# microsoft/GenerativeImage2Text

Hardware: AMD Instinct MI355X
Metric: captions/sec whole-node (GIT_BASE 224px bs=64/GPU greedy len=20) (higher is better)
Workload: dtype f16; 1 GPU; GIT_BASE 224px bs=64/GPU greedy max_len=20 frames=1; global_batch=64, parallelism=dp1, decode_steps_per_caption=19, seq_len_returned=20, hip_graph=True, contexts_in_flight=4, layernorm_folded=True, library=libgitmi_f16.so, encoder_chains=2, schedule=mixed

## Files before the change

### generativeimage2text_amd/csrc/kernels_attn_decode.hip

```cpp
#include "gitmi_common.h"
#include "launchers.h"
#include "dgemm_shared.h"
#include <algorithm>
#include <type_traits>

#pragma clang fp contract(off)

namespace gitmi {

static constexpr int HD = 64;

__global__ __launch_bounds__(256) void kv_repack_frag_kernel(const bf16_t* __restrict__ qkv, bf16_t* __restrict__ kf,
                                                             bf16_t* __restrict__ vt, int N, int Np, int H, int d) {
    __shared__ bf16_t vs[32][HD + 8];
    const int s = blockIdx.x, h = blockIdx.y, b = blockIdx.z, tid = threadIdx.x;
    const int nsteps = Np >> 5;
    bf16_t* kdst = kf + ((size_t)b * H + h) * Np * HD;
    bf16_t* vdst = vt + ((size_t)b * H + h) * Np * HD;
    const int key = tid >> 3, ch = tid & 7;
    const int n = s * 32 + key;
    u32x4_t kv = {0u, 0u, 0u, 0u}, vv = kv;
    if (n < N) {
        const bf16_t* src = qkv + ((size_t)b * N + n) * 3 * d + d + h * HD + ch * 8;
        kv = *reinterpret_cast<const u32x4_t*>(src);
        vv = *reinterpret_cast<const u32x4_t*>(src + d);
    }
    *reinterpret_cast<u32x4_t*>(kdst + frag_tile(n >> 4, ch >> 2, 2, (ch & 3) * 16 + (n & 15))) = kv;
    *reinterpret_cast<u32x4_t*>(&vs[key][ch * 8]) = vv;
    __syncthreads();
    const int dt = tid >> 6, lane = tid & 63, lg = lane >> 4, dim = dt * 16 + (lane & 15);
    bf16_t o[8];
#pragma unroll
    for (int e = 0; e < 8; ++e) o[e] = vs[(e >> 2) * 16 + lg * 4 + (e & 3)][dim];
    u32x4_t ov;
#pragma unroll
    for (int e = 0; e < 4; ++e) ov[e] = (uint32_t)o[2 * e] | ((uint32_t)o[2 * e + 1] << 16);
    *reinterpret_cast<u32x4_t*>(vdst + (((size_t)s * 4 + dt) * 64 + lane) * 8) = ov;
}

__device__ __forceinline__ void unpack8(const u32x4_t& r, float (&v)[8]) {
#pragma unroll
    for (int i = 0; i < 4; ++i) {
        unpack2op(r[i], v[2 * i], v[2 * i + 1]);
    }
}
__device__ __forceinline__ void ld8bf(const bf16_t* p, float (&v)[8]) { unpack8(*reinterpret_cast<const u32x4_t*>(p), v); }

constexpr int ACS = 4;

struct Pair {
    int h, row0;
    bool on;
};

struct QkvSrc {
    const bf16_t* q0;
    int row_stride, part;
    __device__ __forceinline__ const bf16_t* q(int j) const { return q0 + (size_t)j * row_stride; }
    __device__ __forceinline__ const bf16_t* k(int j) const { return q(j) + part; }
    __device__ __forceinline__ const bf16_t* v(int j) const { return q(j) + 2 * part; }
};
__device__ __forceinline__ QkvSrc qkv_rows(const AttnDecodeArgs& a, const Pair& p) {
    return QkvSrc{reinterpret_cast<const bf16_t*>(a.qkv) + (size_t)p.row0 * (3 * a.d) + p.h * HD, 3 * a.d, a.d};
}

template <int KB>
__device__ __forceinline__ void load_text_kv(const AttnDecodeArgs& a, const Pair& p, const QkvSrc& qs, int j, int s, int sub, u32x4_t& kr, u32x4_t& vr) {
    if (s == a.pos) {
        kr = *reinterpret_cast<const u32x4_t*>(qs.k(j) + sub * 8);
        vr = *reinterpret_cast<const u32x4_t*>(qs.v(j) + sub * 8);
    } else {
        const int srow = KB == 1 ? p.row0 : a.kv_src[(size_t)(p.row0 + j) * a.ld_src + s];
        const size_t off = ((size_t)srow * a.T_max + s) * a.d + p.h * HD + sub * 8;
        kr = *reinterpret_cast<const u32x4_t*>(reinterpret_cast<const bf16_t*>(a.txt_k) + off);
        vr = *reinterpret_cast<const u32x4_t*>(reinterpret_cast<const bf16_t*>(a.txt_v) + off);
    }
}

template <int KB, int TI>
struct TextItems {
    int j[TI];
    u32x4_t kr[TI], vr[TI];
    __device__ __forceinline__ void load(const AttnDecodeArgs& a, const Pair& p, const QkvSrc& qs, int grp, int ngrp, int sub) {
        const int nt = a.pos + 1;
#pragma unroll
        for (int u = 0; u < TI; ++u) {
            const int it = grp + ngrp * u;
            j[u] = (p.on && it < a.beams * nt) ? it / nt : -1;
            const int s = it < a.beams * nt ? it % nt : 0;
            kr[u] = u32x4_t{0u, 0u, 0u, 0u};
            vr[u] = kr[u];
            if (j[u] >= 0) load_text_kv<KB>(a, p, qs, j[u], s, sub, kr[u], vr[u]);
        }
    }
};

__device__ __forceinline__ void append_text_cache(const AttnDecodeArgs& a, const Pair& p, const QkvSrc& qs, int t, int sub) {
    if (p.on && t < a.beams * 8) {
        const int j = t >> 3;
        const size_t dst = ((size_t)(p.row0 + j) * a.T_max + a.pos) * a.d + p.h * HD + sub * 8;
        *reinterpret_cast<u32x4_t*>(reinterpret_cast<bf16_t*>(a.txt_k) + dst) = *reinterpret_cast<const u32x4_t*>(qs.k(j) + sub * 8);
        *reinterpret_cast<u32x4_t*>(reinterpret_cast<bf16_t*>(a.txt_v) + dst) = *reinterpret_cast<const u32x4_t*>(qs.v(j) + sub * 8);
    }
}

__device__ __forceinline__ void load_q_frag(const AttnDecodeArgs& a, const Pair& p, const QkvSrc& qs, int l15, int lg, bf16x8_t (&qf)[2]) {
#pragma unroll
    for (int ds = 0; ds < 2; ++ds) {
        float qv[8] = {0.f, 0.f, 0.f, 0.f, 0.f, 0.f, 0.f, 0.f};
        if (p.on && l15 < a.beams)
            ld8bf(qs.q(l15) + ds * 32 + lg * 8, qv);
        u32x4_t t;
#pragma unroll
        for (int e = 0; e < 4; ++e) t[e] = pack2bf(qv[2 * e] * a.scale, qv[2 * e + 1] * a.scale);
        qf[ds] = __builtin_bit_cast(bf16x8_t, t);
    }
}

struct ImagePartial {
    float m, l;
    f32x4_t o[4];
    __device__ __forceinline__ void init() {
        m = -INFINITY;
        l = 0.f;
#pragma unroll
        for (int dt = 0; dt < 4; ++dt) o[dt] = f32x4_t{0.f, 0.f, 0.f, 0.f};
    }
    __device__ __forceinline__ static void mask_max(f32x4_t (&sc)[2], int s, int nimg_steps, int n_img, int lg, float& cm) {
#pragma unroll
        for (int t = 0; t < 2; ++t)
#pragma unroll
            for (int r = 0; r < 4; ++r) {
                if (s * 32 + t * 16 + lg * 4 + r >= n_img || s >= nimg_steps) sc[t][r] = -INFINITY;
                cm = fmaxf(cm, sc[t][r]);
            }
    }
    __device__ __forceinline__ float new_max(float cm, bool rescale) {
        cm = fmaxf(cm, __shfl_xor(cm, 16, 64));
        cm = fmaxf(cm, __shfl_xor(cm, 32, 64));
        const float mn = fmaxf(m, cm);
        if (rescale) {
            const float al = fast_exp(m - mn);
            l *= al;
#pragma unroll
            for (int dt = 0; dt < 4; ++dt) { o[dt][0] *= al; o[dt][1] *= al; o[dt][2] *= al; o[dt][3] *= al; }
        }
        m = mn;
        return mn;
    }
    __device__ __forceinline__ bf16x8_t p_frag(const f32x4_t (&sc)[2], float mn) {
        float p[8];
#pragma unroll
        for (int t = 0; t < 2; ++t)
#pragma unroll
            for (int r = 0; r < 4; ++r) {
                p[t * 4 + r] = fast_exp(sc[t][r] - mn);
                l += p[t * 4 + r];
            }
        u32x4_t pp;
#pragma unroll
        for (int e = 0; e < 4; ++e) pp[e] = pack2bf(p[2 * e], p[2 * e + 1]);
        return __builtin_bit_cast(bf16x8_t, pp);
    }
    __device__ __forceinline__ void finish() {
        l += __shfl_xor(l, 16, 64);
        l += __shfl_xor(l, 32, 64);
    }
    template <int KB>
    __device__ __forceinline__ void publish(float (&slot)[KB][HD + 2], int k, int l15, int lg) const {
        if (l15 < k) {
#pragma unroll
            for (int dt = 0; dt < 4; ++dt)
#pragma unroll
                for (int r = 0; r < 4; ++r) slot[l15][dt * 16 + lg * 4 + r] = o[dt][r];
            if (lg == 0) { slot[l15][HD] = m; slot[l15][HD + 1] = l; }
        }
    }
};

template <int KB>
struct TextPartial {
    float q[KB][8], m[KB], l[KB], o[KB][8];
    __device__ __forceinline__ void init(const AttnDecodeArgs& a, const Pair& p, const QkvSrc& qs, int sub) {
#pragma unroll
        for (int j = 0; j < KB; ++j) {
            m[j] = -INFINITY;
            l[j] = 0.f;
#pragma unroll
            for (int e = 0; e < 8; ++e) { q[j][e] = 0.f; o[j][e] = 0.f; }
            if (p.on && j < a.beams) {
                ld8bf(qs.q(j) + sub * 8, q[j]);
#pragma unroll
                for (int e = 0; e < 8; ++e) q[j][e] *= a.scale;
            }
        }
    }
    __device__ __forceinline__ void item(int jj, const u32x4_t& kr, const u32x4_t& vr) {
        float kv[8], vv[8];
        unpack8(kr, kv);
        unpack8(vr, vv);
#pragma unroll
        for (int j = 0; j < KB; ++j) {
            if (j == jj) {
                float sv = 0.f;
#pragma unroll
                for (int e = 0; e < 8; ++e) sv = fmaf(q[j][e], kv[e], sv);
                sv += __shfl_xor(sv, 1, 64);
                sv += __shfl_xor(sv, 2, 64);
                sv += __shfl_xor(sv, 4, 64);
                const float mn = fmaxf(m[j], sv);
                const float al = fast_exp(m[j] - mn);
                const float pe = fast_exp(sv - mn);
                l[j] = fmaf(l[j], al, pe);
#pragma unroll
                for (int e = 0; e < 8; ++e) o[j][e] = fmaf(o[j][e], al, pe * vv[e]);
                m[j] = mn;
            }
        }
    }
    template <int TI>
    __device__ __forceinline__ void items(const TextItems<KB, TI>& ti, bool enabled) {
#pragma unroll
        for (int u = 0; u < TI; ++u) {
            if (ti.j[u] >= 0 && enabled) item(ti.j[u], ti.kr[u], ti.vr[u]);
        }
    }
    template <int TI>
    __device__ __forceinline__ void tail(const AttnDecodeArgs& a, const Pair& p, const QkvSrc& qs, int grp, int ngrp, int sub) {
        if (!p.on) return;
        const int nt = a.pos + 1;
        for (int it = grp + ngrp * TI; it < a.beams * nt; it += ngrp) {
            u32x4_t kr, vr;
            load_text_kv<KB>(a, p, qs, it / nt, it % nt, sub, kr, vr);
            item(it / nt, kr, vr);
        }
    }
    __device__ __forceinline__ void merge_groups() {
#pragma unroll
        for (int j = 0; j < KB; ++j) {
#pragma unroll
            for (int off = 8; off < 64; off <<= 1) {
                const float m2 = __shfl_xor(m[j], off, 64);
                const float l2 = __shfl_xor(l[j], off, 64);
                const float mn = fmaxf(m[j], m2);
                const float a1 = m[j] == -INFINITY ? 0.f : fast_exp(m[j] - mn);
                const float a2 = m2 == -INFINITY ? 0.f : fast_exp(m2 - mn);
                l[j] = fmaf(l[j], a1, l2 * a2);
#pragma unroll
                for (int e = 0; e < 8; ++e) {
                    const float o2 = __shfl_xor(o[j][e], off, 64);
                    o[j][e] = fmaf(o[j][e], a1, o2 * a2);
                }
                m[j] = mn;
            }
        }
    }
    __device__ __forceinline__ void fold_into(float (&slot)[KB][HD + 2], int k, int lane, int sub) const {
#pragma unroll
        for (int j = 0; j < KB; ++j) {
            if (lane < 8 && j < k) {
                const float mi = slot[j][HD], li = slot[j][HD + 1];
                const float mn = fmaxf(mi, m[j]);
                const float a1 = mi == -INFINITY ? 0.f : fast_exp(mi - mn);
                const float a2 = m[j] == -INFINITY ? 0.f : fast_exp(m[j] - mn);
#pragma unroll
                for (int e = 0; e < 8; ++e) slot[j][sub * 8 + e] = fmaf(slot[j][sub * 8 + e], a1, o[j][e] * a2);
                if (sub == 0) { slot[j][HD] = mn; slot[j][HD + 1] = fmaf(li, a1, l[j] * a2); }
            }
        }
    }
};

__device__ __forceinline__ void store_out(const AttnDecodeArgs& a, int row, int col, float r) {
    bf16_t* O = reinterpret_cast<bf16_t*>(a.out);
    if (a.out_frag) O[frag_offset(row, col, a.d >> 5)] = f2bf(r);
    else O[(size_t)row * a.d + col] = f2bf(r);
}
template <int KB>
__device__ __forceinline__ void write_rows(const AttnDecodeArgs& a, const Pair& p, const float (&s0)[KB][HD + 2], int t, int nthr) {
    if (!p.on) return;
    for (int i = t; i < a.beams * HD; i += nthr) {
        const int j = i / HD, dd = i % HD;
        const float r1 = s0[j][dd] / s0[j][HD + 1];
        store_out(a, p.row0 + j, p.h * HD + dd, r1);
    }
}
template <int KB>
__device__ __forceinline__ void write_rows(const AttnDecodeArgs& a, const Pair& p, const float (&s0)[KB][HD + 2],
                                           const float (&s1)[KB][HD + 2], int t, int nthr) {
    if (!p.on) return;
    for (int i = t; i < a.beams * HD; i += nthr) {
        const int j = i / HD, dd = i % HD;
        const float m0 = s0[j][HD], m1 = s1[j][HD];
        const float mm = fmaxf(m0, m1);
        const float a0 = m0 == -INFINITY ? 0.f : fast_exp(m0 - mm);
        const float a1 = m1 == -INFINITY ? 0.f : fast_exp(m1 - mm);
        const float num = fmaf(a0, s0[j][dd], a1 * s1[j][dd]);
        const float den = fmaf(a0, s0[j][HD + 1], a1 * s1[j][HD + 1]);
        const float r = num / den;
        store_out(a, p.row0 + j, p.h * HD + dd, r);
    }
}

template <int KB, int TI = 3, int PW = 1, int NH = 2, bool RAGGED = false>
__global__ __launch_bounds__(64 * NH * PW) void attn_decode_mfma_kernel(AttnDecodeArgs a) {
    __shared__ float part[PW][NH][KB][HD + 2];
    constexpr int PT = 64 * NH;

    const int tid = threadIdx.x, lane = tid & 63, wave = tid >> 6;
    const int l15 = lane & 15, lg = lane >> 4;
    const int hp = wave / NH, half = wave % NH;
    const int H = a.d / HD;
    const int k = a.beams;
    const int Np = a.N_pad, nsteps = Np >> 5;
    const int pair = NH == 2 ? (int)(blockIdx.y * H + blockIdx.x) : (int)blockIdx.x * PW + hp;
    Pair p;
    p.on = PW == 1 || pair < a.n_pairs;
    p.h = p.on ? pair % H : 0;
    const int b = p.on ? pair / H : 0;
    p.row0 = b * k;
    const int bi = a.img_of ? a.img_of[b] : b;
    const bf16_t* Kf = reinterpret_cast<const bf16_t*>(a.img_k) + ((size_t)bi * H + p.h) * Np * HD;
    const bf16_t* Vt = reinterpret_cast<const bf16_t*>(a.img_v) + ((size_t)bi * H + p.h) * Np * HD;
    const int n_img = RAGGED ? a.ntok[bi] : a.N_img;
    const int nimg_steps = (!p.on || (a.dbg & 1)) ? 0 : RAGGED ? (n_img + 31) >> 5 : nsteps;

    bf16x8_t kq[ACS][2][2], vq[ACS][4];
    auto load_chunk = [&](int s0) {
#pragma unroll
        for (int c = 0; c < ACS; ++c) {
            const int s = s0 + NH * c;
            const bool on = s < nimg_steps && !(a.dbg & 8);
            const bf16_t* kp = Kf + frag_tile(2 * s, 0, 2, lane);
            const bf16_t* vp = Vt + ((size_t)s * 4 * 64 + lane) * 8;
#pragma unroll
            for (int t = 0; t < 2; ++t)
#pragma unroll
                for (int ds = 0; ds < 2; ++ds) {
                    const bf16x8_t* q = reinterpret_cast<const bf16x8_t*>(kp + (t * 2 + ds) * 512);
                    kq[c][t][ds] = !on ? bf16x8_t{0, 0, 0, 0, 0, 0, 0, 0} : (a.dbg & 16) ? *q : __builtin_nontemporal_load(q);
                }
#pragma unroll
            for (int dt = 0; dt < 4; ++dt) {
                const bf16x8_t* q = reinterpret_cast<const bf16x8_t*>(vp + dt * 512);
                vq[c][dt] = !on ? bf16x8_t{0, 0, 0, 0, 0, 0, 0, 0} : (a.dbg & 16) ? *q : __builtin_nontemporal_load(q);
            }
        }
    };
    load_chunk(half);

    const int t = tid % PT, grp = t >> 3, sub = tid & 7;
    const QkvSrc qs = qkv_rows(a, p);
    TextItems<KB, TI> ti;
    ti.load(a, p, qs, grp, 8 * NH, sub);
    append_text_cache(a, p, qs, t, sub);
    bf16x8_t qf[2];
    load_q_frag(a, p, qs, l15, lg, qf);

    ImagePartial ip;
    ip.init();
    for (int s0 = half; s0 < nimg_steps; s0 += NH * ACS) {
        if (s0 != half) load_chunk(s0);
        f32x4_t sc[ACS][2];
        float cm = -INFINITY;
#pragma unroll
        for (int c = 0; c < ACS; ++c) {
#pragma unroll
            for (int u = 0; u < 2; ++u) {
                sc[c][u] = mfma16(kq[c][u][0], qf[0], f32x4_t{0.f, 0.f, 0.f, 0.f});
                sc[c][u] = mfma16(kq[c][u][1], qf[1], sc[c][u]);
            }
            ip.mask_max(sc[c], s0 + NH * c, nimg_steps, RAGGED ? n_img : a.N_img, lg, cm);
        }
        const float mn = ip.new_max(cm, s0 != half);
#pragma unroll
        for (int c = 0; c < ACS; ++c) {
            const bf16x8_t pf = ip.p_frag(sc[c], mn);
            if (a.dbg & 4) {
#pragma unroll
                for (int dt = 0; dt < 4; ++dt) asm volatile("" ::"v"(vq[c][dt]));
                asm volatile("" ::"v"(pf));
                continue;
            }
#pragma unroll
            for (int dt = 0; dt < 4; ++dt) ip.o[dt] = mfma16(vq[c][dt], pf, ip.o[dt]);
        }
    }
    ip.finish();
    TextPartial<KB> tp;
    tp.init(a, p, qs, sub);
    tp.items(ti, !(a.dbg & 2));
    tp.template tail<TI>(a, p, qs, grp, 8 * NH, sub);
    tp.merge_groups();
    ip.publish(part[hp][half], k, l15, lg);
    if constexpr (NH > 1) __syncthreads(); else __builtin_amdgcn_wave_barrier();
    tp.fold_into(part[hp][half], k, lane, sub);
    if constexpr (NH > 1) __syncthreads(); else __builtin_amdgcn_wave_barrier();
    if constexpr (NH == 1) write_rows(a, p, part[hp][0], t, PT);
    else write_rows(a, p, part[hp][0], part[hp][NH - 1], t, PT);
}

constexpr int AQ_PW = 8;
constexpr int AQ_STRIPS = 3 * HD / 16;

__device__ __forceinline__ void attn_lds_barrier() {
    asm volatile("s_waitcnt lgkmcnt(0)" ::: "memory");
    __builtin_amdgcn_s_barrier();
    asm volatile("" ::: "memory");
}

template <int TI>
__global__ __launch_bounds__(64 * AQ_PW) void attn_decode_qkv_kernel(AttnDecodeArgs a) {
    constexpr int KB = 1;
    __shared__ __attribute__((aligned(16))) f32x4_t red[AQ_STRIPS][4][1][64];
    __shared__ __attribute__((aligned(16))) bf16_t rows[AQ_PW][3 * HD];
    __shared__ float part[AQ_PW][KB][HD + 2];

    const int tid = threadIdx.x, lane = tid & 63;
    const int wave = __builtin_amdgcn_readfirstlane(tid >> 6);
    const int l15 = lane & 15, lg = lane >> 4;
    const int H = a.d / HD, B = a.n_pairs / H;
    const int Np = a.N_pad, nsteps = Np >> 5;
    const int nsb = (B + AQ_PW - 1) / AQ_PW, total = H * nsb, per = (total + 7) >> 3;
    const int blk = (int)(blockIdx.x & 7) * per + (int)(blockIdx.x >> 3);
    if (blk >= total) return;
    const int b0 = (blk % nsb) * AQ_PW;
    Pair p;
    p.h = blk / nsb;
    p.on = b0 + wave < B;
    const int b = p.on ? b0 + wave : 0;
    p.row0 = b;
    const int bi = a.img_of ? a.img_of[b] : b;
    const bf16_t* Kf = reinterpret_cast<const bf16_t*>(a.img_k) + ((size_t)bi * H + p.h) * Np * HD;
    const bf16_t* Vt = reinterpret_cast<const bf16_t*>(a.img_v) + ((size_t)bi * H + p.h) * Np * HD;
    const int nimg_steps = p.on ? nsteps : 0;

    bf16x8_t kq[ACS][2][2], vq[ACS][4];
    auto load_k = [&](int s0) {
#pragma unroll
        for (int c = 0; c < ACS; ++c) {
            const bool on = s0 + c < nimg_steps;
            const bf16_t* kp = Kf + frag_tile(2 * (s0 + c), 0, 2, lane);
#pragma unroll
            for (int t = 0; t < 2; ++t)
#pragma unroll
                for (int ds = 0; ds < 2; ++ds)
                    kq[c][t][ds] = !on ? bf16x8_t{0, 0, 0, 0, 0, 0, 0, 0}
                                       : __builtin_nontemporal_load(reinterpret_cast<const bf16x8_t*>(kp + (t * 2 + ds) * 512));
        }
    };
    auto load_v = [&](int s0) {
#pragma unroll
        for (int c = 0; c < ACS; ++c) {
            const bool on = s0 + c < nimg_steps;
            const bf16_t* vp = Vt + ((size_t)(s0 + c) * 4 * 64 + lane) * 8;
#pragma unroll
            for (int dt = 0; dt < 4; ++dt)
                vq[c][dt] = !on ? bf16x8_t{0, 0, 0, 0, 0, 0, 0, 0}
                                : __builtin_nontemporal_load(reinterpret_cast<const bf16x8_t*>(vp + dt * 512));
        }
    };
    load_k(0);

    const int ksteps = a.d >> 5, N = 3 * a.d;
    const int slice = wave & 3;
    const KSlice ks = k_slice(ksteps, 4, slice);
    const int rt = b0 >> 4;
    auto strip_of = [&](int ls) { return (ls >> 2) * (a.d >> 4) + p.h * 4 + (ls & 3); };
    bf16x8_t xf[DW_KS][1];
    load_x_slice(xf, reinterpret_cast<const bf16_t*>(a.x), rt, ks, ksteps, lane);
#pragma unroll 2
    for (int u = 0; u < AQ_STRIPS / 2; ++u) {
        const int ls = (wave >> 2) * (AQ_STRIPS / 2) + u;
        const WSlice wf = load_w_slice<false>(reinterpret_cast<const bf16_t*>(a.w), strip_of(ls), ks, ksteps, lane);
        f32x4_t acc[1] = {f32x4_t{0.f, 0.f, 0.f, 0.f}};
        mfma_slice(acc, wf, xf, ks);
        red[ls][slice][0][lane] = acc[0];
    }
    load_v(0);
    const int fm_raw = rt * 16 + l15;
    const int fm = fm_raw < a.M ? fm_raw : a.M - 1;
    const bool second = wave + AQ_PW < AQ_STRIPS;
    const int fn0 = strip_of(wave) * 16 + lg * 4, fn1 = strip_of(second ? wave + AQ_PW : wave) * 16 + lg * 4;
    RowStatLoads sl;
    if (a.stats_in) stats_issue(sl, a.stats_in, a.strips_in, a.M, fm, lg);
    const float4 bias4[2] = {load_cols4(a.bias, fn0, N), load_cols4(a.bias, fn1, N)};
    float4 cs4[2] = {float4{0.f, 0.f, 0.f, 0.f}, float4{0.f, 0.f, 0.f, 0.f}};
    if (a.stats_in) { cs4[0] = load_cols4(a.colsum, fn0, N); cs4[1] = load_cols4(a.colsum, fn1, N); }
    attn_lds_barrier();
    {
#pragma clang fp contract(fast)
        float mean = 0.f, rstd = 1.f;
        if (a.stats_in) stats_finish(sl, a.inv_d, a.eps_in, mean, rstd);
        const int i = l15 - (b0 & 15);
#pragma unroll
        for (int t = 0; t < 2; ++t) {
            if (t == 1 && !second) break;
            const int ls = wave + t * AQ_PW;
            const f32x4_t tot = sum_waves<4>(red[ls], 0, lane);
            DGEMM_CONSUMER_FINISH(v, tot, bias4[t], cs4[t], a.stats_in, mean, rstd, GITMI_ACT_NONE);
            if (i >= 0 && i < AQ_PW) {
                uint2 o;
                o.x = pack2bf(v[0], v[1]);
                o.y = pack2bf(v[2], v[3]);
                *reinterpret_cast<uint2*>(&rows[i][ls * 16 + lg * 4]) = o;
            }
        }
    }
    attn_lds_barrier();
    const QkvSrc qs{rows[wave], 0, HD};

    const int grp = lane >> 3, sub = lane & 7;
    TextItems<KB, TI> ti;
    ti.load(a, p, qs, grp, 8, sub);
    append_text_cache(a, p, qs, lane, sub);
    bf16x8_t qf[2];
    load_q_frag(a, p, qs, l15, lg, qf);

    ImagePartial ip;
    ip.init();
    for (int s0 = 0; s0 < nimg_steps; s0 += ACS) {
        if (s0 != 0) { load_k(s0); load_v(s0); }
        f32x4_t sc[ACS][2];
        float cm = -INFINITY;
#pragma unroll
        for (int c = 0; c < ACS; ++c) {
#pragma unroll
            for (int u = 0; u < 2; ++u) {
                sc[c][u] = mfma16(kq[c][u][0], qf[0], f32x4_t{0.f, 0.f, 0.f, 0.f});
                sc[c][u] = mfma16(kq[c][u][1], qf[1], sc[c][u]);
            }
            ip.mask_max(sc[c], s0 + c, nimg_steps, a.N_img, lg, cm);
        }
        const float mn = ip.new_max(cm, s0 != 0);
#pragma unroll
        for (int c = 0; c < ACS; ++c) {
            const bf16x8_t pf = ip.p_frag(sc[c], mn);
#pragma unroll
            for (int dt = 0; dt < 4; ++dt) ip.o[dt] = mfma16(vq[c][dt], pf, ip.o[dt]);
        }
    }
    ip.finish();
    TextPartial<KB> tp;
    tp.init(a, p, qs, sub);
    tp.items(ti, true);
    tp.template tail<TI>(a, p, qs, grp, 8, sub);
    tp.merge_groups();
    ip.publish(part[wave], a.beams, l15, lg);
    __builtin_amdgcn_wave_barrier();
    tp.fold_into(part[wave], a.beams, lane, sub);
    __builtin_amdgcn_wave_barrier();
    write_rows(a, p, part[wave], lane, 64);
}

typedef __attribute__((address_space(3))) void attn_lds_void_t;

template <int N> __device__ __forceinline__ void attn_wait_vm() { asm volatile("s_waitcnt vmcnt(%0)" ::"n"(N) : "memory"); }
__device__ __forceinline__ void attn_wait_slots_ahead(int ahead) {
    switch (ahead) {
        case 0: attn_wait_vm<0>(); break;
        case 1: attn_wait_vm<4>(); break;
        case 2: attn_wait_vm<8>(); break;
        case 3: attn_wait_vm<12>(); break;
        case 4: attn_wait_vm<16>(); break;
        case 5: attn_wait_vm<20>(); break;
        case 6: attn_wait_vm<24>(); break;
        case 7: attn_wait_vm<28>(); break;
        case 8: attn_wait_vm<32>(); break;
        case 9: attn_wait_vm<36>(); break;
        case 10: attn_wait_vm<40>(); break;
        default: attn_wait_vm<44>(); break;
    }
}

constexpr int AS_WAVES = 4;
constexpr int AS_SLOT = 4096;

template <int KB, int TI, int RING>
__global__ __launch_bounds__(64 * AS_WAVES) void attn_decode_stream_kernel(AttnDecodeArgs a) {
    static_assert(RING >= 2 && RING <= 12, "ring depth");
    __shared__ __attribute__((aligned(16))) unsigned char ring_mem[AS_WAVES][RING * AS_SLOT];
    __shared__ float part[AS_WAVES][KB][HD + 2];

    const int tid = threadIdx.x, lane = tid & 63;
    const int wave = __builtin_amdgcn_readfirstlane(tid >> 6);
    const int l15 = lane & 15, lg = lane >> 4;
    const int H = a.d / HD;
    const int k = a.beams;
    const int Np = a.N_pad, nsteps = Np >> 5;
    unsigned char* ring = ring_mem[wave];

    const int W = (int)gridDim.x * AS_WAVES, w0 = (int)blockIdx.x * AS_WAVES + wave;
    const int npw = w0 < a.n_pairs ? (a.n_pairs - 1 - w0) / W + 1 : 0;
    const int slots_per_pair = 2 * nsteps;
    const int total_slots = npw * slots_per_pair;

    int issued = 0;
    int p_ord = 0, p_s0 = 0, p_v = 0, p_c = 0;
    const bf16_t* p_K = nullptr; const bf16_t* p_V = nullptr;
    auto producer_pair = [&]() {
        const int pair = w0 + p_ord * W;
        const int h = pair % H, b = pair / H;
        const int bi = a.img_of ? a.img_of[b] : b;
        p_K = reinterpret_cast<const bf16_t*>(a.img_k) + ((size_t)bi * H + h) * Np * HD;
        p_V = reinterpret_cast<const bf16_t*>(a.img_v) + ((size_t)bi * H + h) * Np * HD;
    };
    if (npw > 0) producer_pair();
    auto issue_slot = [&]() {
        if (issued >= total_slots) return;
        const bf16_t* src = (p_v ? p_V : p_K) + (size_t)(p_s0 + p_c) * (AS_SLOT / 2) + lane * 8;
        unsigned char* dst = ring + (issued % RING) * AS_SLOT;
#pragma unroll
        for (int f = 0; f < 4; ++f)
            __builtin_amdgcn_global_load_lds((const void*)(src + f * 512), (attn_lds_void_t*)(dst + f * 1024), 16, 0, 2);
        ++issued;
        const int nsc = min(ACS, nsteps - p_s0);
        if (++p_c == nsc) {
            p_c = 0;
            if (p_v == 0) p_v = 1;
            else {
                p_v = 0; p_s0 += ACS;
                if (p_s0 >= nsteps) { p_s0 = 0; ++p_ord; if (p_ord < npw) producer_pair(); }
            }
        }
    };
    for (int i = 0; i < RING; ++i) issue_slot();

    int consumed = 0;
    auto slot_ready = [&]() -> const unsigned char* {
        const int ahead = issued - consumed - 1;
        if (ahead == RING - 1) attn_wait_vm<4 * (RING - 1)>();
        else attn_wait_slots_ahead(ahead);
        return ring + (consumed % RING) * AS_SLOT;
    };
    auto slot_done = [&]() {
        asm volatile("s_waitcnt lgkmcnt(0)" ::: "memory");
        ++consumed;
        issue_slot();
    };


    for (int ord = 0; ord < npw; ++ord) {
        const int pair = w0 + ord * W;
        const Pair p{pair % H, (pair / H) * k, true};

        const int grp = lane >> 3, sub = lane & 7;
        const QkvSrc qs = qkv_rows(a, p);
        TextItems<KB, TI> ti;
        ti.load(a, p, qs, grp, 8, sub);
        append_text_cache(a, p, qs, lane, sub);
        bf16x8_t qf[2];
        load_q_frag(a, p, qs, l15, lg, qf);

        ImagePartial ip;
        ip.init();
        for (int s0 = 0; s0 < nsteps; s0 += ACS) {
            f32x4_t sc[ACS][2];
            float cm = -INFINITY;
#pragma unroll
            for (int c = 0; c < ACS; ++c) {
                if (s0 + c < nsteps) {
                    const unsigned char* sl = slot_ready();
                    bf16x8_t kq[2][2];
#pragma unroll
                    for (int t = 0; t < 2; ++t)
#pragma unroll
                        for (int ds = 0; ds < 2; ++ds)
                            kq[t][ds] = *reinterpret_cast<const bf16x8_t*>(sl + (t * 2 + ds) * 1024 + lane * 16);
                    __builtin_amdgcn_sched_barrier(0);
#pragma unroll
                    for (int t = 0; t < 2; ++t) {
                        sc[c][t] = mfma16(kq[t][0], qf[0], f32x4_t{0.f, 0.f, 0.f, 0.f});
                        sc[c][t] = mfma16(kq[t][1], qf[1], sc[c][t]);
                    }
                    slot_done();
                } else {
                    sc[c][0] = f32x4_t{0.f, 0.f, 0.f, 0.f};
                    sc[c][1] = sc[c][0];
                }
                ip.mask_max(sc[c], s0 + c, nsteps, a.N_img, lg, cm);
            }
            const float mn = ip.new_max(cm, s0 != 0);
#pragma unroll
            for (int c = 0; c < ACS; ++c) {
                const bf16x8_t pf = ip.p_frag(sc[c], mn);
                if (s0 + c < nsteps) {
                    const unsigned char* sl = slot_ready();
                    bf16x8_t vq[4];
#pragma unroll
                    for (int dt = 0; dt < 4; ++dt) vq[dt] = *reinterpret_cast<const bf16x8_t*>(sl + dt * 1024 + lane * 16);
                    __builtin_amdgcn_sched_barrier(0);
#pragma unroll
                    for (int dt = 0; dt < 4; ++dt) ip.o[dt] = mfma16(vq[dt], pf, ip.o[dt]);
                    slot_done();
                } else {
#pragma unroll
                    for (int dt = 0; dt < 4; ++dt) ip.o[dt] = mfma16(bf16x8_t{0, 0, 0, 0, 0, 0, 0, 0}, pf, ip.o[dt]);
                }
            }
        }
        ip.finish();
        TextPartial<KB> tp;
        tp.init(a, p, qs, sub);
        tp.items(ti, true);
        tp.template tail<TI>(a, p, qs, grp, 8, sub);
        tp.merge_groups();
        ip.publish(part[wave], k, l15, lg);
        __builtin_amdgcn_wave_barrier();
        tp.fold_into(part[wave], k, lane, sub);
        __builtin_amdgcn_wave_barrier();
        write_rows(a, p, part[wave], lane, 64);
        __builtin_amdgcn_wave_barrier();
    }
}

hipError_t launch_kv_repack_frag(const void* qkv, void* kf, void* vt, int B, int N, int N_pad, int H, int d, hipStream_t s) {
    if (B <= 0 || N <= 0) return hipSuccess;
    if (N_pad % 32 || N_pad < N) return hipErrorInvalidValue;
    hipLaunchKernelGGL(kv_repack_frag_kernel, dim3(N_pad / 32, H, B), dim3(256), 0, s, (const bf16_t*)qkv, (bf16_t*)kf,
                       (bf16_t*)vt, N, N_pad, H, d);
    return hipGetLastError();
}

template <typename F>
static void with_beam_rows(int beams, F&& f) {
    if (beams <= 1) f(std::integral_constant<int, 1>{});
    else if (beams <= 2) f(std::integral_constant<int, 2>{});
    else if (beams <= 4) f(std::integral_constant<int, 4>{});
    else f(std::integral_constant<int, 8>{});
}

int attn_decode_pairs_per_wg(const AttnDecodeArgs& a, int B, int H) {
    int pw = a.pairs_per_wg >= 8 ? 8 : a.pairs_per_wg >= 4 || a.pairs_per_wg <= 0 ? 4 : a.pairs_per_wg >= 2 ? 2 : 1;
    while (pw > 1 && B * H / pw < 96) pw >>= 1;
    if (a.beams > 4 && pw == 8) pw = 4;
    return pw;
}

bool attn_decode_qkv_form(const AttnDecodeArgs& a, int B, int H) {
    if (B <= 0 || a.beams != 1 || a.waves_per_pair == 2 || a.ntok || a.stream_wgs != 0 || a.dbg) return false;
    if (a.N_img < 1 || a.N_pad % 32 || a.N_pad < a.N_img || a.N_pad > 8 * 32) return false;
    if (a.d != H * HD || a.d > 4 * DW_KS * 32 || a.M < B) return false;
    if (!a.x || !a.w || !a.bias) return false;
    return !a.stats_in || (a.colsum && a.strips_in >= 1 && a.strips_in <= 4 * STRIP_SLOTS);
}

hipError_t launch_attn_decode_qkv(const AttnDecodeArgs& a, int B, int H, hipStream_t s) {
    if (!attn_decode_qkv_form(a, B, H)) return hipErrorInvalidValue;
    AttnDecodeArgs p = a;
    p.n_pairs = B * H;
    const int total = H * ((B + AQ_PW - 1) / AQ_PW);
    hipLaunchKernelGGL((attn_decode_qkv_kernel<3>), dim3(8 * ((total + 7) / 8)), dim3(64 * AQ_PW), 0, s, p);
    return hipGetLastError();
}

hipError_t launch_attn_decode_mfma(const AttnDecodeArgs& a, int B, int H, hipStream_t s) {
    if (B <= 0) return hipSuccess;
    if (a.beams > 8 || a.N_pad % 32 || a.N_pad < a.N_img || a.N_img < 1) return hipErrorInvalidValue;
    if (a.ntok && a.stream_wgs > 0) return hipErrorInvalidValue;
    AttnDecodeArgs p = a;
    p.n_pairs = B * H;
    if (a.stream_wgs > 0) {
        const int nwg = std::max(1, std::min(a.stream_wgs, (p.n_pairs + AS_WAVES - 1) / AS_WAVES));
        with_beam_rows(a.beams, [&](auto kb) {
            constexpr int KB = decltype(kb)::value;
            hipLaunchKernelGGL((attn_decode_stream_kernel<KB, 3, KB == 8 ? 8 : 9>), dim3(nwg), dim3(64 * AS_WAVES), 0, s, p);
        });
        return hipGetLastError();
    }
    const bool one_wave = a.waves_per_pair == 1 || (a.waves_per_pair != 2 && a.N_pad <= 8 * 32);
    if (a.ntok || !one_wave) {
        with_beam_rows(a.beams, [&](auto kb) {
            constexpr int KB = decltype(kb)::value;
            if (a.ntok) hipLaunchKernelGGL((attn_decode_mfma_kernel<KB, 3, 1, 2, true>), dim3(H, B), dim3(128), 0, s, p);
            else hipLaunchKernelGGL((attn_decode_mfma_kernel<KB>), dim3(H, B), dim3(128), 0, s, p);
        });
        return hipGetLastError();
    }
    const int pw = attn_decode_pairs_per_wg(a, B, H);
    with_beam_rows(a.beams, [&](auto kb) {
        constexpr int KB = decltype(kb)::value;
        auto packed = [&](auto pwc) {
            constexpr int PW = decltype(pwc)::value;
            hipLaunchKernelGGL((attn_decode_mfma_kernel<KB, 3, PW, 1>), dim3((p.n_pairs + PW - 1) / PW), dim3(64 * PW), 0, s, p);
        };
        if (pw == 8) { if constexpr (KB < 8) packed(std::integral_constant<int, 8>{}); }
        else if (pw == 4) packed(std::integral_constant<int, 4>{});
        else if (pw == 2) packed(std::integral_constant<int, 2>{});
        else packed(std::integral_constant<int, 1>{});
    });
    return hipGetLastError();
}

}
```

Measured before the change: 11700 captions/s.

## Overlap first K/V chunk loads with fused QKV projection via LDS DMA

In the fused QKV-projection plus decode-attention kernel, the first image K chunk is now prefetched. Part of it is DMA'd straight into per-wave LDS slots through global_load_lds, and the rest is loaded into registers, all issued before the projection MFMAs. The W slices and epilogue constants are also hoisted ahead of those MFMAs. Loads for out-of-range steps are always issued against a dummy address, so fixed vmcnt waits can be used, and the results are masked to zero at use. The aim is to hide global latency of K/V behind the GEMM, at the cost of extra LDS (8 waves × 3 × 4KB), more live registers and more complex wait accounting.

```diff
diff --git a/generativeimage2text_amd/csrc/kernels_attn_decode.hip b/generativeimage2text_amd/csrc/kernels_attn_decode.hip
--- a/generativeimage2text_amd/csrc/kernels_attn_decode.hip
+++ b/generativeimage2text_amd/csrc/kernels_attn_decode.hip
@@ -402,6 +402,19 @@
 
 constexpr int AQ_PW = 8;
 constexpr int AQ_STRIPS = 3 * HD / 16;
+constexpr int AQ_LDS_STEPS = 3;
+constexpr int AS_SLOT = 4096;
+typedef __attribute__((address_space(3))) void attn_lds_void_t;
+
+template <int N>
+__device__ __forceinline__ void attn_wait_vm_only() {
+    static_assert(N >= 0 && N < 64, "vmcnt is a 6-bit counter");
+    __builtin_amdgcn_sched_barrier(0);
+    asm volatile("" ::: "memory");
+    __builtin_amdgcn_s_waitcnt((N & 15) | ((N >> 4) << 14) | (7 << 4) | (15 << 8));
+    asm volatile("" ::: "memory");
+    __builtin_amdgcn_sched_barrier(0);
+}
 
 __device__ __forceinline__ void attn_lds_barrier() {
     asm volatile("s_waitcnt lgkmcnt(0)" ::: "memory");
@@ -409,12 +422,14 @@
     asm volatile("" ::: "memory");
 }
 
-template <int TI>
+template <int TI, bool OVL = true>
 __global__ __launch_bounds__(64 * AQ_PW) void attn_decode_qkv_kernel(AttnDecodeArgs a) {
     constexpr int KB = 1;
+    static_assert(AQ_LDS_STEPS < ACS, "the chunk's last step stays in registers");
     __shared__ __attribute__((aligned(16))) f32x4_t red[AQ_STRIPS][4][1][64];
     __shared__ __attribute__((aligned(16))) bf16_t rows[AQ_PW][3 * HD];
     __shared__ float part[AQ_PW][KB][HD + 2];
+    __shared__ __attribute__((aligned(16))) unsigned char kslot[OVL ? AQ_PW : 1][OVL ? AQ_LDS_STEPS * AS_SLOT : 16];
 
     const int tid = threadIdx.x, lane = tid & 63;
     const int wave = __builtin_amdgcn_readfirstlane(tid >> 6);
@@ -436,57 +451,109 @@
     const int nimg_steps = p.on ? nsteps : 0;
 
     bf16x8_t kq[ACS][2][2], vq[ACS][4];
-    auto load_k = [&](int s0) {
-#pragma unroll
-        for (int c = 0; c < ACS; ++c) {
+    const bf16x8_t zero8 = {0, 0, 0, 0, 0, 0, 0, 0};
+    auto load_frag = [&](const bf16_t* q, bool on, auto always_issue) -> bf16x8_t {
+        if constexpr (decltype(always_issue)::value) return __builtin_nontemporal_load(reinterpret_cast<const bf16x8_t*>(q));
+        else return !on ? zero8 : __builtin_nontemporal_load(reinterpret_cast<const bf16x8_t*>(q));
+    };
+    auto frag_used = [&](const bf16x8_t& f, int s) -> bf16x8_t { return OVL && s >= nimg_steps ? zero8 : f; };
+    auto load_k = [&](int s0, auto c0, auto always_issue) {
+#pragma unroll
+        for (int c = decltype(c0)::value; c < ACS; ++c) {
             const bool on = s0 + c < nimg_steps;
             const bf16_t* kp = Kf + frag_tile(2 * (s0 + c), 0, 2, lane);
 #pragma unroll
             for (int t = 0; t < 2; ++t)
 #pragma unroll
                 for (int ds = 0; ds < 2; ++ds)
-                    kq[c][t][ds] = !on ? bf16x8_t{0, 0, 0, 0, 0, 0, 0, 0}
-                                       : __builtin_nontemporal_load(reinterpret_cast<const bf16x8_t*>(kp + (t * 2 + ds) * 512));
-        }
-    };
-    auto load_v = [&](int s0) {
+                    kq[c][t][ds] = load_frag(decltype(always_issue)::value && !on ? Kf : kp + (t * 2 + ds) * 512, on, always_issue);
+        }
+    };
+    auto load_v = [&](int s0, auto always_issue) {
 #pragma unroll
         for (int c = 0; c < ACS; ++c) {
             const bool on = s0 + c < nimg_steps;
             const bf16_t* vp = Vt + ((size_t)(s0 + c) * 4 * 64 + lane) * 8;
 #pragma unroll
             for (int dt = 0; dt < 4; ++dt)
-                vq[c][dt] = !on ? bf16x8_t{0, 0, 0, 0, 0, 0, 0, 0}
-                                : __builtin_nontemporal_load(reinterpret_cast<const bf16x8_t*>(vp + dt * 512));
-        }
-    };
-    load_k(0);
+                vq[c][dt] = load_frag(decltype(always_issue)::value && !on ? Vt : vp + dt * 512, on, always_issue);
+        }
+    };
+    constexpr std::integral_constant<int, 0> all_steps{};
+    constexpr std::integral_constant<int, OVL ? AQ_LDS_STEPS : 0> reg_steps{};
+    constexpr std::false_type as_needed{};
+    constexpr std::integral_constant<bool, OVL> fixed_count{};
+    auto dma_k = [&]() {
+#pragma unroll
+        for (int c = 0; c < AQ_LDS_STEPS; ++c) {
+            const bool on = c < nimg_steps;
+            const bf16_t* src = Kf + frag_tile(2 * c, 0, 2, lane);
+#pragma unroll
+            for (int f = 0; f < 4; ++f)
+                __builtin_amdgcn_global_load_lds((const void*)(on ? src + f * 512 : Kf), (attn_lds_void_t*)(kslot[wave] + (c * 4 + f) * 1024), 16, 0, 2);
+        }
+    };
+    auto read_slot = [&]() {
+#pragma unroll
+        for (int c = 0; c < AQ_LDS_STEPS; ++c)
+#pragma unroll
+            for (int t = 0; t < 2; ++t)
+#pragma unroll
+                for (int ds = 0; ds < 2; ++ds)
+                    kq[c][t][ds] = *reinterpret_cast<const bf16x8_t*>(kslot[wave] + (c * 4 + t * 2 + ds) * 1024 + lane * 16);
+    };
+    if constexpr (!OVL) load_k(0, all_steps, as_needed);
 
     const int ksteps = a.d >> 5, N = 3 * a.d;
     const int slice = wave & 3;
     const KSlice ks = k_slice(ksteps, 4, slice);
     const int rt = b0 >> 4;
     auto strip_of = [&](int ls) { return (ls >> 2) * (a.d >> 4) + p.h * 4 + (ls & 3); };
-    bf16x8_t xf[DW_KS][1];
-    load_x_slice(xf, reinterpret_cast<const bf16_t*>(a.x), rt, ks, ksteps, lane);
-#pragma unroll 2
-    for (int u = 0; u < AQ_STRIPS / 2; ++u) {
-        const int ls = (wave >> 2) * (AQ_STRIPS / 2) + u;
-        const WSlice wf = load_w_slice<false>(reinterpret_cast<const bf16_t*>(a.w), strip_of(ls), ks, ksteps, lane);
-        f32x4_t acc[1] = {f32x4_t{0.f, 0.f, 0.f, 0.f}};
-        mfma_slice(acc, wf, xf, ks);
-        red[ls][slice][0][lane] = acc[0];
-    }
-    load_v(0);
     const int fm_raw = rt * 16 + l15;
     const int fm = fm_raw < a.M ? fm_raw : a.M - 1;
     const bool second = wave + AQ_PW < AQ_STRIPS;
     const int fn0 = strip_of(wave) * 16 + lg * 4, fn1 = strip_of(second ? wave + AQ_PW : wave) * 16 + lg * 4;
     RowStatLoads sl;
-    if (a.stats_in) stats_issue(sl, a.stats_in, a.strips_in, a.M, fm, lg);
-    const float4 bias4[2] = {load_cols4(a.bias, fn0, N), load_cols4(a.bias, fn1, N)};
-    float4 cs4[2] = {float4{0.f, 0.f, 0.f, 0.f}, float4{0.f, 0.f, 0.f, 0.f}};
-    if (a.stats_in) { cs4[0] = load_cols4(a.colsum, fn0, N); cs4[1] = load_cols4(a.colsum, fn1, N); }
+    float4 bias4[2], cs4[2] = {float4{0.f, 0.f, 0.f, 0.f}, float4{0.f, 0.f, 0.f, 0.f}};
+    auto load_epilogue_constants = [&]() {
+        if (a.stats_in) stats_issue(sl, a.stats_in, a.strips_in, a.M, fm, lg);
+        bias4[0] = load_cols4(a.bias, fn0, N);
+        bias4[1] = load_cols4(a.bias, fn1, N);
+        if (a.stats_in) { cs4[0] = load_cols4(a.colsum, fn0, N); cs4[1] = load_cols4(a.colsum, fn1, N); }
+    };
+    bf16x8_t xf[DW_KS][1];
+    load_x_slice(xf, reinterpret_cast<const bf16_t*>(a.x), rt, ks, ksteps, lane);
+    if constexpr (OVL) {
+        WSlice wf[AQ_STRIPS / 2];
+#pragma unroll
+        for (int u = 0; u < AQ_STRIPS / 2; ++u)
+            wf[u] = load_w_slice<false>(reinterpret_cast<const bf16_t*>(a.w), strip_of((wave >> 2) * (AQ_STRIPS / 2) + u), ks, ksteps, lane);
+        load_epilogue_constants();
+        __builtin_amdgcn_sched_barrier(0);
+        dma_k();
+        load_k(0, reg_steps, fixed_count);
+        __builtin_amdgcn_sched_barrier(0);
+        attn_wait_vm_only<4 * AQ_LDS_STEPS + 4 * (ACS - AQ_LDS_STEPS)>();
+#pragma unroll
+        for (int u = 0; u < AQ_STRIPS / 2; ++u) {
+            const int ls = (wave >> 2) * (AQ_STRIPS / 2) + u;
+            f32x4_t acc[1] = {f32x4_t{0.f, 0.f, 0.f, 0.f}};
+            mfma_slice(acc, wf[u], xf, ks);
+            red[ls][slice][0][lane] = acc[0];
+        }
+        load_v(0, fixed_count);
+    } else {
+#pragma unroll 2
+        for (int u = 0; u < AQ_STRIPS / 2; ++u) {
+            const int ls = (wave >> 2) * (AQ_STRIPS / 2) + u;
+            const WSlice wf = load_w_slice<false>(reinterpret_cast<const bf16_t*>(a.w), strip_of(ls), ks, ksteps, lane);
+            f32x4_t acc[1] = {f32x4_t{0.f, 0.f, 0.f, 0.f}};
+            mfma_slice(acc, wf, xf, ks);
+            red[ls][slice][0][lane] = acc[0];
+        }
+        load_v(0, as_needed);
+        load_epilogue_constants();
+    }
     attn_lds_barrier();
     {
 #pragma clang fp contract(fast)
@@ -509,6 +576,10 @@
     }
     attn_lds_barrier();
     const QkvSrc qs{rows[wave], 0, HD};
+    if constexpr (OVL) {
+        attn_wait_vm_only<4 * ACS>();
+        read_slot();
+    }
 
     const int grp = lane >> 3, sub = lane & 7;
     TextItems<KB, TI> ti;
@@ -520,15 +591,15 @@
     ImagePartial ip;
     ip.init();
     for (int s0 = 0; s0 < nimg_steps; s0 += ACS) {
-        if (s0 != 0) { load_k(s0); load_v(s0); }
+        if (s0 != 0) { load_k(s0, all_steps, as_needed); load_v(s0, as_needed); }
         f32x4_t sc[ACS][2];
         float cm = -INFINITY;
 #pragma unroll
         for (int c = 0; c < ACS; ++c) {
 #pragma unroll
             for (int u = 0; u < 2; ++u) {
-                sc[c][u] = mfma16(kq[c][u][0], qf[0], f32x4_t{0.f, 0.f, 0.f, 0.f});
-                sc[c][u] = mfma16(kq[c][u][1], qf[1], sc[c][u]);
+                sc[c][u] = mfma16(frag_used(kq[c][u][0], s0 + c), qf[0], f32x4_t{0.f, 0.f, 0.f, 0.f});
+                sc[c][u] = mfma16(frag_used(kq[c][u][1], s0 + c), qf[1], sc[c][u]);
             }
             ip.mask_max(sc[c], s0 + c, nimg_steps, a.N_img, lg, cm);
         }
@@ -537,7 +608,7 @@
         for (int c = 0; c < ACS; ++c) {
             const bf16x8_t pf = ip.p_frag(sc[c], mn);
 #pragma unroll
-            for (int dt = 0; dt < 4; ++dt) ip.o[dt] = mfma16(vq[c][dt], pf, ip.o[dt]);
+            for (int dt = 0; dt < 4; ++dt) ip.o[dt] = mfma16(frag_used(vq[c][dt], s0 + c), pf, ip.o[dt]);
         }
     }
     ip.finish();
@@ -552,8 +623,6 @@
     __builtin_amdgcn_wave_barrier();
     write_rows(a, p, part[wave], lane, 64);
 }
-
-typedef __attribute__((address_space(3))) void attn_lds_void_t;
 
 template <int N> __device__ __forceinline__ void attn_wait_vm() { asm volatile("s_waitcnt vmcnt(%0)" ::"n"(N) : "memory"); }
 __device__ __forceinline__ void attn_wait_slots_ahead(int ahead) {
@@ -574,7 +643,6 @@
 }
 
 constexpr int AS_WAVES = 4;
-constexpr int AS_SLOT = 4096;
 
 template <int KB, int TI, int RING>
 __global__ __launch_bounds__(64 * AS_WAVES) void attn_decode_stream_kernel(AttnDecodeArgs a) {
@@ -738,7 +806,7 @@
 }
 
 bool attn_decode_qkv_form(const AttnDecodeArgs& a, int B, int H) {
-    if (B <= 0 || a.beams != 1 || a.waves_per_pair == 2 || a.ntok || a.stream_wgs != 0 || a.dbg) return false;
+    if (B <= 0 || a.beams != 1 || a.waves_per_pair == 2 || a.ntok || a.stream_wgs != 0 || (a.dbg & ~32)) return false;
     if (a.N_img < 1 || a.N_pad % 32 || a.N_pad < a.N_img || a.N_pad > 8 * 32) return false;
     if (a.d != H * HD || a.d > 4 * DW_KS * 32 || a.M < B) return false;
     if (!a.x || !a.w || !a.bias) return false;
@@ -750,7 +818,14 @@
     AttnDecodeArgs p = a;
     p.n_pairs = B * H;
     const int total = H * ((B + AQ_PW - 1) / AQ_PW);
-    hipLaunchKernelGGL((attn_decode_qkv_kernel<3>), dim3(8 * ((total + 7) / 8)), dim3(64 * AQ_PW), 0, s, p);
+    const dim3 grid(8 * ((total + 7) / 8)), block(64 * AQ_PW);
+#ifdef GITMI_EXPERIMENT
+    if (a.dbg & 32) {
+        hipLaunchKernelGGL((attn_decode_qkv_kernel<3, false>), grid, block, 0, s, p);
+        return hipGetLastError();
+    }
+#endif
+    hipLaunchKernelGGL((attn_decode_qkv_kernel<3>), grid, block, 0, s, p);
     return hipGetLastError();
 }
 
```

New measurement: 11770 captions/s (median of 6 runs). About the same (+0.6%).
